# michaelbzms/DeepRecommendation

Measured on AMD Instinct MI355X. Metric: scored user-item pairs/sec, higher is better.
Workload: dtype f32; 1 GPU; cfg2: BasicNCF 1M users x 100k items, emb_dim=64, batch=65536/GPU, fp32, MLP 128-256-128-1; parallelism=replicas x1 (tables+MLP replicated, batch split, no collective), step_form=HIP-graph launches of 20 steps over the resident index batches, full=False

## Files before the change

deeprecommendation_amd/csrc/mlp_partial.hip:

```cpp
#include "mlp_fused.h"

#ifndef NCF_PART_WD
#define NCF_PART_WD 8
#endif
#ifndef NCF_PART_PF
#define NCF_PART_PF 2
#endif
#ifndef NCF_PART_HYBRID_MAX_PERMILLE
#define NCF_PART_HYBRID_MAX_PERMILLE 500
#endif

namespace ncf {

struct PartialBuildArgs {
    const float* tabA; int64_t rowsA; int64_t ldA; int QA;
    const float* Wp1; const float* b1;
    float* P; int64_t ldP;
};

template <int N1>
__global__ __launch_bounds__(256) void layer1_partial_kernel(PartialBuildArgs a) {
    constexpr int NT1 = N1 / 32;
    const int lane = threadIdx.x & 63;
    const int m = lane & 31, h = lane >> 5;
    const int64_t tile = (int64_t)blockIdx.x * 4 + (threadIdx.x >> 6);
    const int64_t rows = a.rowsA + 1;
    if (tile * 32 >= rows) return;
    const int64_t r = tile * 32 + m;
    const bool ok = r < a.rowsA;
    const float* rowA = a.tabA + (ok ? r : 0) * a.ldA + 4 * h;
    const float zA = ok ? 1.f : 0.f;

    f32x16 acc[NT1];
#pragma unroll
    for (int nt = 0; nt < NT1; ++nt)
#pragma unroll
        for (int g = 0; g < 4; ++g) {
            const f32x4 bb = fused_ldg4(a.b1 + 32 * nt + 8 * g + 4 * h);
            acc[nt][4 * g + 0] = bb[0]; acc[nt][4 * g + 1] = bb[1];
            acc[nt][4 * g + 2] = bb[2]; acc[nt][4 * g + 3] = bb[3];
        }
    const f32x4* wp = reinterpret_cast<const f32x4*>(a.Wp1) + lane;
    f32x4 w[NT1], x;
#pragma unroll
    for (int nt = 0; nt < NT1; ++nt) w[nt] = wp[nt * 64];
    x = fused_ldg4(rowA);
    for (int q = 0; q < a.QA; ++q) {
        f32x4 wn[NT1], xn;
        if (q + 1 < a.QA) {
#pragma unroll
            for (int nt = 0; nt < NT1; ++nt) wn[nt] = wp[((q + 1) * NT1 + nt) * 64];
            xn = fused_ldg4(rowA + 8 * (q + 1));
        }
        const f32x4 xb = x * zA;
#pragma unroll
        for (int nt = 0; nt < NT1; ++nt)
#pragma unroll
            for (int j = 0; j < 4; ++j)
                acc[nt] = __builtin_amdgcn_mfma_f32_32x32x2f32(w[nt][j], xb[j], acc[nt], 0, 0, 0);
#pragma unroll
        for (int nt = 0; nt < NT1; ++nt) w[nt] = wn[nt];
        x = xn;
    }
    if (r >= rows) return;
    float* dst = a.P + r * a.ldP + 4 * h;
#pragma unroll
    for (int nt = 0; nt < NT1; ++nt)
#pragma unroll
        for (int g = 0; g < 4; ++g) {
            f32x4 v;
            v[0] = acc[nt][4 * g + 0]; v[1] = acc[nt][4 * g + 1];
            v[2] = acc[nt][4 * g + 2]; v[3] = acc[nt][4 * g + 3];
            *reinterpret_cast<f32x4*>(dst + 32 * nt + 8 * g) = v;
        }
}

struct PartialArgs {
    const float* P; int64_t rowsA; int64_t ldP;
    const float* tabB; int64_t rowsB; int64_t ldB;
    const int64_t* idxA; const int64_t* idxB;
    int64_t B; int QA;
    const float* Wp1; const float* Wp2; const float* b2;
    const float* wl; const float* bl;
    float* out; int32_t* oob;
};

template <int QB, int N1, int N2>
__global__ __launch_bounds__(256, 2) void score_fused_partial_f32_kernel(PartialArgs a) {
    constexpr int NT1 = N1 / 32;
    constexpr int S = NT1 * QB;
    constexpr int WD0 = (QB >= 16 && N1 >= 256) ? 4 : NCF_PART_WD;
    constexpr int WD = WD0 < S ? WD0 : S;
    constexpr int PF = NCF_PART_PF < 1 ? 1 : (NCF_PART_PF < NT1 ? NCF_PART_PF : NT1);
    const int lane = threadIdx.x & 63;
    const int m = lane & 31, h = lane >> 5;
    const int64_t tile = (int64_t)blockIdx.x * 4 + (threadIdx.x >> 6);
    if (tile * 32 >= a.B) return;
    const int64_t p = tile * 32 + m;
    const int64_t pc = p < a.B ? p : a.B - 1;

    const int64_t ia = a.idxA ? a.idxA[pc] : pc;
    const int64_t ib = a.idxB ? a.idxB[pc] : pc;
    const bool okA = (ia >= 0) & (ia < a.rowsA), okB = (ib >= 0) & (ib < a.rowsB);
    if (!(okA & okB) && a.oob) *a.oob = 1;
    const float* prow = a.P + (okA ? ia : a.rowsA) * a.ldP + 4 * h;
    const float* rowB = a.tabB + (okB ? ib : 0) * a.ldB + 4 * h;
    const float zB = okB ? 1.f : 0.f;

    f32x16 acc1[NT1];
    auto load_p = [&](int nt) {
#pragma unroll
        for (int g = 0; g < 4; ++g) {
            const f32x4 v = fused_ldg4(prow + 32 * nt + 8 * g);
            acc1[nt][4 * g + 0] = v[0]; acc1[nt][4 * g + 1] = v[1];
            acc1[nt][4 * g + 2] = v[2]; acc1[nt][4 * g + 3] = v[3];
        }
    };
    const f32x4* wp = reinterpret_cast<const f32x4*>(a.Wp1) + (int64_t)a.QA * NT1 * 64 + lane;
    auto wfrag = [&](int s) { return wp[((s % QB) * NT1 + s / QB) * 64]; };
    f32x4 w[WD], x[QB];
    load_p(0);
#pragma unroll
    for (int s = 0; s < WD - 1; ++s) w[s] = wfrag(s);
#pragma unroll
    for (int t = 0; t < QB; ++t) x[t] = fused_ldg4(rowB + 8 * t);
#pragma unroll
    for (int nt = 1; nt < PF; ++nt) load_p(nt);
#pragma unroll
    for (int nt = 0; nt < NT1; ++nt) {
#pragma unroll
        for (int t = 0; t < QB; ++t) {
            const int s = nt * QB + t;
            const f32x4 xb = x[t] * zB;
#pragma unroll
            for (int j = 0; j < 4; ++j)
                acc1[nt] = __builtin_amdgcn_mfma_f32_32x32x2f32(w[s % WD][j], xb[j], acc1[nt], 0, 0, 0);
            if (s + WD - 1 < S) w[(s + WD - 1) % WD] = wfrag(s + WD - 1);
        }
        if (nt + PF < NT1) load_p(nt + PF);
#pragma unroll
        for (int t = 0; t < QB; ++t) {
            __builtin_amdgcn_sched_group_barrier(0x008, 4, 0);
            __builtin_amdgcn_sched_group_barrier(0x020, 1, 0);
        }
        __builtin_amdgcn_sched_group_barrier(0x020, 4, 0);
        __builtin_amdgcn_sched_barrier(0);
    }

    float score;
    if constexpr (N2 > 0) {
        f32x16 acc2[N2 / 32];
        fused_layer2<N1, N2>(acc1, acc2, a.b2, a.Wp2, lane);
        score = fused_last_layer(acc2, a.wl, a.bl, lane);
    } else {
        score = fused_last_layer(acc1, a.wl, a.bl, lane);
    }
    if (h == 0 && p < a.B) a.out[p] = score;
}

template <int QB, int N1, int N2>
static void launch_partial(const PartialArgs& a, hipStream_t s) {
    const int64_t tiles = (a.B + 31) / 32;
    hipLaunchKernelGGL((score_fused_partial_f32_kernel<QB, N1, N2>), dim3((unsigned)((tiles + 3) / 4)), dim3(256), 0, s, a);
}

#define NCF_PARTIAL_INSTANCES(X) \
    X(4, 256, 128) X(8, 256, 128) X(12, 256, 128) X(16, 256, 128) \
    X(4, 256, 0) X(8, 256, 0) X(12, 256, 0) X(16, 256, 0) \
    X(4, 128, 0) X(8, 128, 0) X(12, 128, 0) X(16, 128, 0) \
    X(4, 128, 64) X(8, 128, 64) X(12, 128, 64)

static bool partial_dispatch(int QB, int N1, int N2, const PartialArgs* a, hipStream_t s) {
#define X(qb, n1, n2) \
    if (QB == qb && N1 == n1 && N2 == n2) { if (a) launch_partial<qb, n1, n2>(*a, s); return true; }
    NCF_PARTIAL_INSTANCES(X)
#undef X
    return false;
}

static bool partial_shape_ok(int dtype, int EA, int EB, int n_layers, const int* dims) {
    if (dtype != NCF_F32 || !dims || EA <= 0 || EB <= 0 || EA % 8 || EB % 8) return false;
    if (!ncf_score_fused_supported(dtype, EA, EB, n_layers, dims)) return false;
    return partial_dispatch(EB / 8, dims[1], n_layers == 3 ? dims[2] : 0, nullptr, nullptr);
}

}

using namespace ncf;

extern "C" int ncf_score_fused_partial_supported(int dtype, int EA, int EB, int n_layers, const int* dims) {
    return partial_shape_ok(dtype, EA, EB, n_layers, dims) ? 1 : 0;
}

extern "C" int ncf_layer1_partial(int dtype, const void* tabA, int64_t rowsA, int64_t ldA, int EA, int EB, int n_layers,
                                  const int* dims, const void* packed, void* P, int64_t ldP, ncf_stream_t stream) {
    if (!partial_shape_ok(dtype, EA, EB, n_layers, dims))
        return fail(NCF_EUNSUPPORTED, "ncf_layer1_partial: no partial kernel for dtype=%d EA=%d EB=%d layers=%d", dtype, EA, EB, n_layers);
    const int N1 = dims[1];
    if (rowsA < 1 || !tabA || !packed || !P) return fail(NCF_EINVAL, "ncf_layer1_partial: bad argument");
    if (ldA < EA || ldA % 4 || ldP < N1 || ldP % 4 || !aligned16(tabA) || !aligned16(P) || !aligned16(packed))
        return fail(NCF_EINVAL, "ncf_layer1_partial: tables must be 16-byte aligned with ld %% 4 == 0");
    const BlobLayout L = blob_layout(dims, n_layers);
    PartialBuildArgs a;
    a.tabA = (const float*)tabA; a.rowsA = rowsA; a.ldA = ldA; a.QA = EA / 8;
    a.Wp1 = (const float*)packed + L.wp1; a.b1 = (const float*)packed + L.b1;
    a.P = (float*)P; a.ldP = ldP;
    const int64_t tiles = (rowsA + 1 + 31) / 32;
    const dim3 grid((unsigned)((tiles + 3) / 4)), block(256);
    if (N1 == 256) hipLaunchKernelGGL(layer1_partial_kernel<256>, grid, block, 0, (hipStream_t)stream, a);
    else hipLaunchKernelGGL(layer1_partial_kernel<128>, grid, block, 0, (hipStream_t)stream, a);
    return check_launch("ncf_layer1_partial");
}

extern "C" int ncf_score_fused_partial(int dtype, const void* P, int64_t ldP, const void* tabA, int64_t rowsA, int64_t ldA,
                                       const void* tabB, int64_t rowsB, int64_t ldB, const int64_t* idxA, const int64_t* idxB,
                                       int64_t B, int EA, int EB, int n_layers, const int* dims, const void* packed, float* out,
                                       int32_t* oob, ncf_stream_t stream) {
    if (!partial_shape_ok(dtype, EA, EB, n_layers, dims))
        return fail(NCF_EUNSUPPORTED, "ncf_score_fused_partial: no partial kernel for dtype=%d EA=%d EB=%d layers=%d", dtype, EA, EB, n_layers);
    if (B == 0) return NCF_OK;
    const int N1 = dims[1];
    if (B < 0 || rowsA < 1 || !P || !tabA || !tabB || !packed || !out) return fail(NCF_EINVAL, "ncf_score_fused_partial: bad argument");
    if (ldA < EA || ldB < EB || ldP < N1 || ldA % 4 || ldB % 4 || ldP % 4 || !aligned16(tabA) || !aligned16(tabB) || !aligned16(P) ||
        !aligned16(packed))
        return fail(NCF_EINVAL, "ncf_score_fused_partial: tables must be 16-byte aligned with ld %% 4 == 0");
    hipStream_t s = (hipStream_t)stream;
    auto plain = [&](int64_t off, int64_t n) {
        return ncf_score_fused(dtype, tabA, rowsA, ldA, tabB, rowsB, ldB, idxA ? idxA + off : nullptr, idxB ? idxB + off : nullptr,
                               n, EA, EB, n_layers, dims, packed, out + off, oob, stream);
    };
    const int64_t tiles = (B + 31) / 32;
    const int64_t round = 4 * (int64_t)num_cus();
    const int64_t full = tiles / round, rem = tiles % round;
    int64_t head = B;
    if (rem > 0 && rem * 1000 <= round * NCF_PART_HYBRID_MAX_PERMILLE && (full == 0 || (idxA && idxB))) head = full * round * 32;
    if (head == 0) return plain(0, B);
    const BlobLayout L = blob_layout(dims, n_layers);
    const float* pk = (const float*)packed;
    PartialArgs a;
    a.P = (const float*)P; a.rowsA = rowsA; a.ldP = ldP;
    a.tabB = (const float*)tabB; a.rowsB = rowsB; a.ldB = ldB;
    a.idxA = idxA; a.idxB = idxB; a.B = head; a.QA = EA / 8;
    a.Wp1 = pk + L.wp1;
    a.Wp2 = n_layers == 3 ? pk + L.wp2 : nullptr; a.b2 = n_layers == 3 ? pk + L.b2 : nullptr;
    a.wl = pk + L.wl; a.bl = pk + L.bl;
    a.out = out; a.oob = oob;
    partial_dispatch(EB / 8, N1, n_layers == 3 ? dims[2] : 0, &a, s);
    const int rc = check_launch("ncf_score_fused_partial");
    if (rc != NCF_OK || head == B) return rc;
    return plain(head, B - head);
}
```

deeprecommendation_amd/native.py:

```python
from __future__ import annotations

import ctypes
import os
from typing import Optional, Sequence

import torch

_HERE = os.path.dirname(os.path.abspath(__file__))
LIB_PATH = os.environ.get("NCF_HIP_LIBRARY") or os.path.join(_HERE, "libncf_hip.so")

NCF_F32, NCF_BF16 = 0, 1
NCF_OK, NCF_EINVAL, NCF_EUNSUPPORTED, NCF_ELAUNCH, NCF_EWORKSPACE = 0, -1, -2, -3, -4
ATT_MLP, ATT_LINEAR, ATT_COS, ATT_MLP_SCALED = 0, 1, 2, 3
ATT_SCALE_LOG2 = 64

_c_i64 = ctypes.c_int64
_c_p = ctypes.c_void_p
_c_int = ctypes.c_int
_c_size = ctypes.c_size_t

SIGNATURES = {
    "ncf_version": (_c_int, []),
    "ncf_last_error": (ctypes.c_char_p, []),
    "ncf_build_arch": (ctypes.c_char_p, []),
    "ncf_build_id": (ctypes.c_char_p, []),
    "ncf_probe_mfma_bf16": (_c_int, [_c_p, _c_int, _c_int, _c_int, _c_p, _c_p, _c_p]),
    "ncf_probe_copy": (_c_int, [_c_p, _c_p, _c_i64, _c_p]),
    "ncf_probe_gather_read": (_c_int, [_c_p, _c_i64, _c_i64, _c_int, _c_p, _c_i64, _c_int, _c_int, _c_p, _c_p]),
    "ncf_set_option": (_c_int, [ctypes.c_char_p, _c_int]),
    "ncf_get_option": (_c_int, [ctypes.c_char_p, _c_p]),
    "ncf_bucket_ids": (_c_int, [_c_p, _c_i64, _c_i64, _c_i64, _c_int, _c_i64, _c_p, _c_p, _c_p, _c_p, _c_p, _c_p]),
    "ncf_bucket_dedup_table_slots": (_c_size, [_c_i64]),
    "ncf_bucket_ids_dedup": (_c_int, [_c_p, _c_i64, _c_i64, _c_i64, _c_int, _c_i64, _c_p, _c_p, _c_i64, _c_p, _c_p, _c_p, _c_p, _c_p, _c_p]),
    "ncf_gather_buckets": (_c_int, [_c_int, _c_p, _c_i64, _c_i64, _c_p, _c_int, _c_i64, _c_int, _c_p, _c_i64, _c_p, _c_p]),
    "ncf_gather_concat": (_c_int, [_c_int, _c_p, _c_i64, _c_i64, _c_p, _c_i64, _c_i64, _c_p, _c_p, _c_i64, _c_int, _c_int,
                                   _c_p, _c_i64, _c_p, _c_p]),
    "ncf_gather_dot": (_c_int, [_c_int, _c_p, _c_i64, _c_i64, _c_p, _c_i64, _c_i64, _c_p, _c_p, _c_i64, _c_int, _c_p, _c_p, _c_p]),
    "ncf_mlp_workspace_bytes": (_c_size, [_c_int, _c_i64, _c_int, _c_p]),
    "ncf_mlp_forward": (_c_int, [_c_int, _c_p, _c_i64, _c_i64, _c_int, _c_p, _c_p, _c_p, _c_p, _c_size, _c_p, _c_i64, _c_p]),
    "ncf_score_fused_supported": (_c_int, [_c_int, _c_int, _c_int, _c_int, _c_p]),
    "ncf_mlp_packed_bytes": (_c_size, [_c_int, _c_int, _c_p]),
    "ncf_mlp_pack": (_c_int, [_c_int, _c_int, _c_p, _c_p, _c_p, _c_p, _c_size, _c_p]),
    "ncf_score_fused": (_c_int, [_c_int, _c_p, _c_i64, _c_i64, _c_p, _c_i64, _c_i64, _c_p, _c_p, _c_i64, _c_int, _c_int,
                                 _c_int, _c_p, _c_p, _c_p, _c_p, _c_p]),
    "ncf_spmm_csr": (_c_int, [_c_int, _c_p, _c_p, _c_i64, _c_p, _c_p, _c_p, _c_i64, _c_i64, _c_int, _c_p, _c_i64, _c_p,
                              _c_i64, _c_p, _c_int, _c_p]),
    "ncf_spmm_csr_dropout": (_c_int, [_c_int, _c_p, _c_p, _c_i64, _c_p, _c_p, _c_p, _c_i64, _c_i64, _c_int, _c_p, _c_i64, _c_p,
                                      _c_i64, _c_p, _c_int, _c_p, ctypes.c_uint32, ctypes.c_float, _c_p]),
    "ncf_degree_accumulate": (_c_int, [_c_p, _c_i64, _c_i64, _c_p, _c_p, _c_p]),
    "ncf_edge_coef": (_c_int, [_c_p, _c_p, _c_p, _c_p, _c_i64, _c_i64, _c_p, _c_p]),
    "ncf_scale_rows": (_c_int, [_c_p, _c_i64, _c_i64, _c_int, ctypes.c_float, _c_p, _c_i64, _c_p]),
    "ncf_attn_forward": (_c_int, [_c_int, _c_p, _c_i64, _c_p, _c_i64, _c_int, _c_p, ctypes.c_float, _c_p, _c_p, _c_p,
                                  _c_i64, _c_i64, _c_p, _c_i64, _c_int, _c_p, _c_p, _c_i64, _c_p, _c_p]),
    "ncf_attn_forward_dropout": (_c_int, [_c_int, _c_p, _c_i64, _c_p, _c_i64, _c_int, _c_p, ctypes.c_float, _c_p, _c_p, _c_p,
                                          _c_i64, _c_i64, _c_p, _c_i64, _c_int, _c_p, _c_p, _c_i64, _c_p, ctypes.c_uint32, ctypes.c_float, _c_p]),
    "ncf_attn_backward": (_c_int, [_c_int, _c_p, _c_i64, _c_p, _c_i64, _c_int, _c_p, _c_p, _c_p, _c_p, _c_i64, _c_i64, _c_p, _c_i64, _c_int,
                                   _c_p, _c_p, _c_i64, _c_p, _c_i64, _c_p, _c_i64, _c_p, _c_p, _c_i64, _c_p, ctypes.c_uint32, ctypes.c_float, _c_p]),
    "ncf_attn_forward_grouped": (_c_int, [_c_int, _c_p, _c_i64, _c_p, _c_i64, _c_int, _c_p, ctypes.c_float, _c_p, _c_p, _c_p,
                                          _c_i64, _c_i64, _c_p, _c_p, _c_p, _c_i64, _c_int, _c_p, _c_i64, _c_int, _c_p, _c_p,
                                          _c_i64, _c_p, _c_p, _c_p]),
    "ncf_group_pairs_workspace_bytes": (_c_size, [_c_i64]),
    "ncf_group_pairs": (_c_int, [_c_p, _c_i64, _c_i64, _c_int, _c_p, _c_p, _c_p, _c_p, _c_size, _c_p, _c_p]),
    "ncf_group_pairs_rows": (_c_int, [_c_p, _c_i64, _c_i64, _c_int, _c_p, _c_p, _c_p, _c_p, _c_p, _c_size, _c_p, _c_p]),
    "ncf_dense_csr_workspace_bytes": (_c_size, [_c_i64]),
    "ncf_dense_csr_rows": (_c_int, [_c_p, _c_i64, _c_i64, _c_i64, _c_int, _c_p, _c_p, _c_p, _c_size, _c_p]),
    "ncf_dense_csr_fill": (_c_int, [_c_p, _c_i64, _c_i64, _c_i64, _c_p, _c_p, _c_p, _c_p, _c_p]),
    "ncf_attn_candidates_supported": (_c_int, [_c_int, _c_int, _c_int]),
    "ncf_attn_candidates_workspace_bytes": (_c_size, [_c_i64]),
    "ncf_attn_candidates": (_c_int, [_c_p, _c_i64, _c_i64, _c_int, _c_p, _c_i64, _c_p, _c_int, _c_p, _c_p, _c_int, _c_p, _c_i64, _c_p, _c_i64,
                                     _c_p, _c_i64, _c_int, _c_p, _c_p, _c_p, _c_p, _c_p, _c_size, _c_p, _c_p]),
    "ncf_attn_candidates_pack_floats": (_c_size, [_c_int, _c_int]),
    "ncf_attn_candidates_packed_workspace_bytes": (_c_size, [_c_i64, _c_int, _c_i64]),
    "ncf_attn_candidates_pack": (_c_int, [_c_p, _c_i64, _c_int, _c_int, _c_p, _c_p]),
    "ncf_attn_candidates_packed": (_c_int, [_c_p, _c_i64, _c_i64, _c_int, _c_p, _c_p, _c_int, _c_p, _c_p, _c_int, _c_p, _c_i64, _c_p, _c_i64,
                                            _c_p, _c_i64, _c_int, _c_p, _c_p, _c_p, _c_p, _c_p, _c_size, _c_p, _c_p]),
    "ncf_attn_split_supported": (_c_int, [_c_int, _c_int, _c_int, _c_int]),
    "ncf_attn_split_workspace_bytes": (_c_size, [_c_i64, _c_int, _c_int]),
    "ncf_attn_forward_split": (_c_int, [_c_int, _c_p, _c_i64, _c_p, _c_i64, _c_int, _c_p, ctypes.c_float, _c_p, _c_p, _c_p,
                                        _c_i64, _c_i64, _c_p, _c_p, _c_p, _c_p, _c_i64, _c_int, _c_p, _c_i64, _c_int, _c_p, _c_p,
                                        _c_i64, _c_int, _c_int, _c_p, _c_size, _c_p]),
    "ncf_attn_tail_supported": (_c_int, [_c_int, _c_int, _c_int, _c_int]),
    "ncf_attn_tail_pack_weight": (_c_int, [_c_p, _c_int, _c_int, _c_p, _c_p]),
    "ncf_attn_tail": (_c_int, [_c_p, _c_i64, _c_int, _c_p, _c_int, _c_p, _c_i64, _c_int, _c_p, _c_p, _c_p, _c_int, _c_p, _c_p, _c_int,
                               _c_p, ctypes.c_float, _c_int, _c_p, _c_i64, _c_p]),
    "ncf_edge_softmax_csr": (_c_int, [_c_p, _c_p, _c_p, _c_p, _c_i64, _c_i64, _c_p, _c_p]),
    "ncf_edge_softmax_segmented_workspace_bytes": (_c_size, [_c_i64, _c_i64]),
    "ncf_edge_softmax_segmented": (_c_int, [_c_p, _c_p, _c_i64, _c_p, _c_i64, _c_p, _c_p, _c_p, _c_i64, _c_p, _c_p, _c_size, _c_p]),
    "ncf_score_fused_partial_supported": (_c_int, [_c_int, _c_int, _c_int, _c_int, _c_p]),
    "ncf_layer1_partial": (_c_int, [_c_int, _c_p, _c_i64, _c_i64, _c_int, _c_int, _c_int, _c_p, _c_p, _c_p, _c_i64, _c_p]),
    "ncf_score_fused_partial": (_c_int, [_c_int, _c_p, _c_i64, _c_p, _c_i64, _c_i64, _c_p, _c_i64, _c_i64, _c_p, _c_p, _c_i64,
                                         _c_int, _c_int, _c_int, _c_p, _c_p, _c_p, _c_p, _c_p]),
    "ncf_score_folded_supported": (_c_int, [_c_int, _c_int, _c_int]),
    "ncf_score_folded": (_c_int, [_c_int, _c_p, _c_i64, _c_i64, _c_p, _c_i64, _c_i64, _c_p, _c_p, _c_i64, _c_int, _c_int, _c_p,
                                  _c_p, _c_p, _c_p]),
    "ncf_linear_forward": (_c_int, [_c_int, _c_p, _c_i64, _c_i64, _c_p, _c_p, _c_int, _c_int, _c_int, _c_p, _c_i64, _c_p]),
    "ncf_gemm_tn_workspace_bytes": (_c_size, [_c_i64, _c_int, _c_int]),
    "ncf_gemm_tn": (_c_int, [_c_p, _c_i64, _c_p, _c_i64, _c_i64, _c_int, _c_int, _c_p, _c_i64, _c_p, _c_size, _c_p]),
    "ncf_colsum_workspace_bytes": (_c_size, [_c_i64, _c_int]),
    "ncf_colsum": (_c_int, [_c_p, _c_i64, _c_i64, _c_int, _c_p, _c_p, _c_size, _c_p]),
    "ncf_relu_backward": (_c_int, [_c_p, _c_i64, _c_p, _c_i64, _c_i64, _c_int, _c_p]),
    "ncf_relu_backward_out": (_c_int, [_c_p, _c_i64, _c_p, _c_i64, _c_p, _c_i64, _c_i64, _c_int, ctypes.c_float, _c_p]),
    "ncf_scatter_add_rows": (_c_int, [_c_p, _c_i64, _c_p, _c_i64, _c_int, _c_p, _c_i64, _c_i64, _c_p, _c_p]),
    "ncf_l2_normalize_rows": (_c_int, [_c_p, _c_i64, _c_i64, _c_int, _c_p, _c_i64, _c_p]),
    "ncf_gather_cols": (_c_int, [_c_p, _c_i64, _c_p, _c_p, _c_i64, _c_int, _c_i64, _c_p, _c_i64, _c_p, _c_p]),
    "ncf_scatter_add_cols": (_c_int, [_c_p, _c_i64, _c_p, _c_i64, _c_int, _c_p, _c_i64, _c_i64, _c_p, _c_p]),
    "ncf_topk_workspace_bytes": (_c_size, [_c_i64, _c_i64, _c_int]),
    "ncf_topk_rows": (_c_int, [_c_p, _c_i64, _c_i64, _c_i64, _c_p, _c_p, _c_int, _c_p, _c_p, _c_p, _c_p, _c_size, _c_p]),
    "ncf_dot_topk_workspace_bytes": (_c_size, [_c_i64, _c_i64, _c_int, _c_int]),
    "ncf_dot_topk": (_c_int, [_c_p, _c_i64, _c_i64, _c_p, _c_i64, _c_i64, _c_p, _c_p, _c_i64, _c_i64, _c_int, _c_p, _c_p, _c_int, _c_p,
                              _c_p, _c_p, _c_p, _c_size, _c_p, _c_p]),
    "ncf_mlp_topk_supported": (_c_int, [_c_int, _c_int, _c_int, _c_int, _c_p, _c_int]),
    "ncf_mlp_topk_workspace_bytes": (_c_size, [_c_i64, _c_i64, _c_int, _c_int, _c_p, _c_int]),
    "ncf_mlp_topk": (_c_int, [_c_int, _c_p, _c_i64, _c_i64, _c_p, _c_i64, _c_i64, _c_int, _c_int, _c_int, _c_p, _c_p, _c_i64, _c_i64,
                              _c_int, _c_p, _c_p, _c_p, _c_p, _c_int, _c_p, _c_p, _c_p, _c_p, _c_size, _c_p, _c_p]),
    "ncf_adam_step": (_c_int, [_c_p, _c_p, _c_p, _c_p, _c_i64, ctypes.c_float, ctypes.c_float, ctypes.c_float, ctypes.c_float,
                               ctypes.c_float, _c_i64, _c_p]),
    "ncf_negative_cdf": (_c_int, [_c_p, _c_i64, _c_p, ctypes.c_float, _c_p, _c_p, _c_p]),
    "ncf_sample_negatives": (_c_int, [_c_p, _c_p, _c_p, _c_i64, _c_p, _c_i64, ctypes.c_uint32, _c_i64, _c_p, _c_p, _c_p]),
}

_lib = None


class NativeError(RuntimeError):
    def __init__(self, code, msg):
        super().__init__(f"libncf_hip: {msg} (status {code})")
        self.code = code


def load_library(path: Optional[str] = None) -> ctypes.CDLL:
    global _lib
    if _lib is not None and path is None:
        return _lib
    p = path or LIB_PATH
    if not os.path.exists(p):
        raise RuntimeError(
            f"{p} not found: the HIP extension is not built. Run `python -c 'import __graft_entry__ as g; g.build()'` "
            "(needs hipcc). deeprecommendation_amd has no CPU fallback.")
    lib = ctypes.CDLL(p)
    for name, (res, args) in SIGNATURES.items():
        fn = getattr(lib, name)
        fn.restype = res
        fn.argtypes = args
    if path is None:
        if not os.environ.get("NCF_HIP_LIBRARY"):
            _check_build_id(lib, p)
        _lib = lib
        _options_from_environment(lib)
    return lib


def _check_build_id(lib, path):
    try:
        from .csrc import build as _build
        want = _build.source_id()
    except (ImportError, OSError):
        return
    have = lib.ncf_build_id().decode()
    if have != want:
        raise RuntimeError(f"{path} is stale: built from sources {have}, the sources here are {want}. "
                           "Rebuild: python -m deeprecommendation_amd.csrc.build")


OPTION_VALUES = {
    "bf16_kernel": {"auto": 0, "ws": 1, "stream": 2, "ws8": 3},
    "linear_kernel": {"auto": 0, "rs": 1, "rsp": 2},
    "linear_kslices": {"auto": 0, "4": 4, "8": 8},
    "attn_grouped_kernel": {"auto": 0, "lds": 1, "scalar": 2},
    "gather_kernel": {"auto": 0, "step": 1, "persistent": 2},
}
_ENV_OPTIONS = {"NCF_BF16_KERNEL": "bf16_kernel", "NCF_LINEAR_KERNEL": "linear_kernel", "NCF_LINEAR_KS": "linear_kslices",
# ... 186 lines not shown
def mlp_forward(x: torch.Tensor, weights: Sequence[torch.Tensor], biases: Sequence[Optional[torch.Tensor]],
                out: Optional[torch.Tensor] = None) -> torch.Tensor:
    lib = load_library()
    _dev(x, "x")
    if x.dtype != torch.float32:
        raise TypeError(f"mlp_forward computes in fp32; got activations of dtype {x.dtype}")
    B, K0, ldx = _rows2d(x, "x")
    dims = [K0] + [int(w.shape[0]) for w in weights]
    for i, w in enumerate(weights):
        _dev(w, "weight")
        if w.dtype != torch.float32 or not w.is_contiguous() or w.shape[1] != dims[i]:
            raise ValueError(f"weight {i} must be contiguous fp32 [{dims[i + 1]}, {dims[i]}]")
    biases = [None if b is None else b.contiguous() for b in biases]
    n = len(weights)
    d = _dims_array(dims)
    ws_bytes = lib.ncf_mlp_workspace_bytes(NCF_F32, B, n, d)
    ws = torch.empty(max(ws_bytes, 1), dtype=torch.uint8, device=x.device)
    if out is None:
        out = torch.empty((B, dims[-1]), dtype=torch.float32, device=x.device)
    _, _, ldo = _rows2d(out, "out")
    _check(lib.ncf_mlp_forward(NCF_F32, _ptr(x), B, ldx, n, d, _ptr_array(weights), _ptr_array(biases), _ptr(ws), ws_bytes,
                               _ptr(out), ldo, _stream(x)))
    return out


def linear(x: torch.Tensor, weight: torch.Tensor, bias: Optional[torch.Tensor] = None, out=None) -> torch.Tensor:
    return mlp_forward(x, [weight], [bias], out=out)


class PackedMLP:

    def __init__(self, weights: Sequence[torch.Tensor], biases: Sequence[Optional[torch.Tensor]], dtype=torch.float32):
        lib = load_library()
        self.dims = [int(weights[0].shape[1])] + [int(w.shape[0]) for w in weights]
        self.n_layers = len(weights)
        self.device = weights[0].device
        self.dtype = dtype
        self.dt = NCF_F32 if dtype == torch.float32 else NCF_BF16
        d = _dims_array(self.dims)
        nbytes = lib.ncf_mlp_packed_bytes(self.dt, self.n_layers, d)
        if nbytes == 0:
            raise NativeError(NCF_EUNSUPPORTED, "MLP shape cannot be packed for the fused kernel")
        ws = [w.detach().to(torch.float32).contiguous() for w in weights]
        bs = [None if b is None else b.detach().to(torch.float32).contiguous() for b in biases]
        for w in ws:
            _dev(w, "weight")
        self.blob = torch.empty(nbytes, dtype=torch.uint8, device=self.device)
        _check(lib.ncf_mlp_pack(self.dt, self.n_layers, d, _ptr_array(ws), _ptr_array(bs), _ptr(self.blob), nbytes,
                                _stream(ws[0])))

    def supports(self, EA: int, EB: int) -> bool:
        return bool(load_library().ncf_score_fused_supported(self.dt, EA, EB, self.n_layers, _dims_array(self.dims)))


def fused_supported(EA: int, EB: int, dims: Sequence[int], dtype=torch.float32) -> bool:
    dt = NCF_F32 if dtype == torch.float32 else NCF_BF16
    return bool(load_library().ncf_score_fused_supported(dt, EA, EB, len(dims) - 1, _dims_array(dims)))


def score_fused(tabA: torch.Tensor, idxA, tabB: Optional[torch.Tensor], idxB, packed: PackedMLP,
                out: Optional[torch.Tensor] = None, B: Optional[int] = None) -> torch.Tensor:
    lib = load_library()
    _dev(tabA, "tabA")
    rowsA, EA, ldA = _rows2d(tabA, "tabA")
    rowsB = EB = ldB = 0
    if tabB is not None:
        _dev(tabB, "tabB")
        rowsB, EB, ldB = _rows2d(tabB, "tabB")
    idxA, idxB = _idx(idxA), _idx(idxB)
    if B is None:
        B = idxA.numel() if idxA is not None else (idxB.numel() if idxB is not None else rowsA)
    if out is None:
        out = torch.empty((B, 1), dtype=torch.float32, device=tabA.device)
    if tabA.dtype != packed.dtype:
        raise TypeError(f"tables are {tabA.dtype} but the MLP was packed for {packed.dtype}")
    _check(lib.ncf_score_fused(_dt(tabA), _ptr(tabA), rowsA, ldA, _ptr(tabB), rowsB, ldB, _ptr(idxA), _ptr(idxB), B, EA, EB,
                               packed.n_layers, _dims_array(packed.dims), _ptr(packed.blob), _ptr(out),
                               _ptr(_oob_flag(tabA.device)), _stream(tabA)))
    return out


def partial_supported(EA: int, EB: int, packed: PackedMLP) -> bool:
    return packed.dt == NCF_F32 and bool(load_library().ncf_score_fused_partial_supported(
        NCF_F32, int(EA), int(EB), packed.n_layers, _dims_array(packed.dims)))


def layer1_partial(tabA: torch.Tensor, packed: PackedMLP, out: Optional[torch.Tensor] = None) -> torch.Tensor:
    lib = load_library()
    _dev(tabA, "tabA")
    rowsA, EA, ldA = _rows2d(tabA, "tabA")
    EB, N1 = packed.dims[0] - EA, packed.dims[1]
    if out is None:
        out = torch.empty((rowsA + 1, N1), dtype=torch.float32, device=tabA.device)
    if out.shape[0] < rowsA + 1 or out.shape[1] < N1:
        raise ValueError(f"layer1_partial: out must hold ({rowsA + 1}, {N1}) floats")
    _, _, ldP = _rows2d(out, "out")
    _check(lib.ncf_layer1_partial(_dt(tabA), _ptr(tabA), rowsA, ldA, EA, EB, packed.n_layers, _dims_array(packed.dims),
                                  _ptr(packed.blob), _ptr(out), ldP, _stream(tabA)))
    return out


def score_fused_partial(P: torch.Tensor, tabA: torch.Tensor, idxA, tabB: torch.Tensor, idxB, packed: PackedMLP,
                        out: Optional[torch.Tensor] = None, B: Optional[int] = None) -> torch.Tensor:
    lib = load_library()
    _dev(tabA, "tabA"), _dev(tabB, "tabB"), _dev(P, "P")
    rowsA, EA, ldA = _rows2d(tabA, "tabA")
    rowsB, EB, ldB = _rows2d(tabB, "tabB")
    _, _, ldP = _rows2d(P, "P")
    if P.dtype != torch.float32 or P.shape[0] != rowsA + 1 or P.shape[1] != packed.dims[1]:
        raise ValueError(f"P must be fp32 ({rowsA + 1}, {packed.dims[1]}), built by layer1_partial from this tabA")
    idxA, idxB = _idx(idxA), _idx(idxB)
    if B is None:
        B = idxA.numel() if idxA is not None else (idxB.numel() if idxB is not None else rowsA)
    if out is None:
        out = torch.empty((B, 1), dtype=torch.float32, device=tabA.device)
    if tabA.dtype != packed.dtype:
        raise TypeError(f"tables are {tabA.dtype} but the MLP was packed for {packed.dtype}")
    _check(lib.ncf_score_fused_partial(_dt(tabA), _ptr(P), ldP, _ptr(tabA), rowsA, ldA, _ptr(tabB), rowsB, ldB, _ptr(idxA),
                                       _ptr(idxB), B, EA, EB, packed.n_layers, _dims_array(packed.dims), _ptr(packed.blob),
                                       _ptr(out), _ptr(_oob_flag(tabA.device)), _stream(tabA)))
    return out


def spmm_csr(segptr: torch.Tensor, row_of: Optional[torch.Tensor], col: torch.Tensor, coef: Optional[torch.Tensor],
             z: torch.Tensor, N: int, y: Optional[torch.Tensor] = None, acc_sum: Optional[torch.Tensor] = None,
             partial: Optional[torch.Tensor] = None, fixup: bool = True, dropout: Optional[tuple] = None) -> torch.Tensor:
    lib = load_library()
    _dev(z, "z")
    Nz, D, ldz = _rows2d(z, "z")
    n_seg = segptr.numel() - 1
    if segptr.dtype != torch.int64 or col.dtype != torch.int32:
        raise TypeError("segptr must be int64 and col int32")
    if row_of is not None and row_of.dtype != torch.int32:
        raise TypeError("row_of must be int32")
    if y is None:
        y = torch.empty((N, D), dtype=torch.float32, device=z.device)
    if row_of is not None and partial is None:
        partial = torch.empty((n_seg, D), dtype=torch.float32, device=z.device)
    if dropout is not None and dropout[0] > 0:
        p, seed, eid = dropout
        if eid is not None and (eid.dtype != torch.int32 or eid.numel() != col.numel()):
            raise TypeError("edge ids must be int32, one per CSR entry")
        _check(lib.ncf_spmm_csr_dropout(NCF_F32, _ptr(segptr), _ptr(row_of), n_seg, _ptr(col), _ptr(coef), _ptr(z), Nz, ldz, D, _ptr(y),
                                        y.stride(0), _ptr(acc_sum), 0 if acc_sum is None else acc_sum.stride(0), _ptr(partial),
                                        1 if fixup else 0, _ptr(eid), int(seed) & 0xFFFFFFFF, float(p), _stream(z)))
        return y
    _check(lib.ncf_spmm_csr(NCF_F32, _ptr(segptr), _ptr(row_of), n_seg, _ptr(col), _ptr(coef), _ptr(z), Nz, ldz, D, _ptr(y),
                            y.stride(0), _ptr(acc_sum), 0 if acc_sum is None else acc_sum.stride(0), _ptr(partial),
                            1 if fixup else 0, _stream(z)))
    return y


class SegmentedCSR:

    def __init__(self, rowptr: torch.Tensor, col: torch.Tensor, coef: Optional[torch.Tensor], seg_len: int = 512, fan: int = 64):
        self.n_rows = rowptr.numel() - 1
        self.col, self.coef = col, coef
        counts = rowptr[1:] - rowptr[:-1]
        self._build_tree(rowptr, counts, seg_len, fan)

    @staticmethod
    def _split(rowptr, row_ids, counts, seg_len):
        dev = rowptr.device
        nseg = torch.clamp((counts + seg_len - 1) // seg_len, min=1)
        n = counts.numel()
        if n == 0 or int(nseg.max()) == 1:
# ... 730 lines not shown
```

include/ncf_abi.h:

```cpp
#ifndef NCF_ABI_H
#define NCF_ABI_H

#include <stddef.h>
#include <stdint.h>

#ifdef __cplusplus
extern "C" {
#endif

#define NCF_ABI_VERSION 1

typedef void* ncf_stream_t;

enum ncf_dtype { NCF_F32 = 0, NCF_BF16 = 1 };

enum ncf_status {
    NCF_OK = 0,
    NCF_EINVAL = -1,
    NCF_EUNSUPPORTED = -2,
    NCF_ELAUNCH = -3,
    NCF_EWORKSPACE = -4
};

int ncf_version(void);
const char* ncf_last_error(void);
const char* ncf_build_arch(void);
const char* ncf_build_id(void);

int ncf_set_option(const char* name, int value);
int ncf_get_option(const char* name, int* value);

int ncf_gather_concat(int dtype,
                      const void* dev_tabA, int64_t rowsA, int64_t ldA,
                      const void* dev_tabB, int64_t rowsB, int64_t ldB,
                      const int64_t* dev_idxA, const int64_t* dev_idxB,
                      int64_t B, int EA, int EB,
                      void* dev_out, int64_t ldOut,
                      int32_t* dev_oob_flag, ncf_stream_t stream);

int ncf_gather_dot(int dtype,
                   const void* dev_tabA, int64_t rowsA, int64_t ldA,
                   const void* dev_tabB, int64_t rowsB, int64_t ldB,
                   const int64_t* dev_idxA, const int64_t* dev_idxB,
                   int64_t B, int E, float* dev_out,
                   int32_t* dev_oob_flag, ncf_stream_t stream);

int ncf_bucket_ids(const int64_t* dev_idx, int64_t B, int64_t rows_per_rank, int64_t total_rows, int world, int64_t cap,
                   int64_t* dev_send, int64_t* dev_slot, int32_t* dev_counts,
                   int32_t* dev_oob_flag, int32_t* dev_overflow_flag, ncf_stream_t stream);

size_t ncf_bucket_dedup_table_slots(int64_t B);
int ncf_bucket_ids_dedup(const int64_t* dev_idx, int64_t B, int64_t rows_per_rank, int64_t total_rows, int world, int64_t cap,
                         int64_t* dev_hkeys, int64_t* dev_hvals, int64_t table_slots,
                         int64_t* dev_send, int64_t* dev_slot, int32_t* dev_counts,
                         int32_t* dev_oob_flag, int32_t* dev_overflow_flag, ncf_stream_t stream);

int ncf_gather_buckets(int dtype, const void* dev_table, int64_t rows, int64_t ld, const int64_t* dev_recv, int world, int64_t cap, int E,
                       void* dev_out, int64_t ldout, int32_t* dev_oob_flag, ncf_stream_t stream);

size_t ncf_mlp_workspace_bytes(int dtype, int64_t B, int n_layers, const int* dims);
int ncf_mlp_forward(int dtype, const void* dev_x, int64_t B, int64_t ldx,
                    int n_layers, const int* dims,
                    const void* const* host_W, const void* const* host_b,
                    void* dev_workspace, size_t workspace_bytes,
                    void* dev_out, int64_t ldOut, ncf_stream_t stream);

int ncf_score_fused_supported(int dtype, int EA, int EB, int n_layers, const int* dims);
size_t ncf_mlp_packed_bytes(int dtype, int n_layers, const int* dims);
int ncf_mlp_pack(int dtype, int n_layers, const int* dims,
                 const void* const* host_W, const void* const* host_b,
                 void* dev_packed, size_t packed_bytes, ncf_stream_t stream);
int ncf_score_fused(int dtype,
                    const void* dev_tabA, int64_t rowsA, int64_t ldA,
                    const void* dev_tabB, int64_t rowsB, int64_t ldB,
                    const int64_t* dev_idxA, const int64_t* dev_idxB,
                    int64_t B, int EA, int EB,
                    int n_layers, const int* dims, const void* dev_packed,
                    float* dev_out, int32_t* dev_oob_flag, ncf_stream_t stream);

int ncf_score_fused_partial_supported(int dtype, int EA, int EB, int n_layers, const int* dims);
int ncf_layer1_partial(int dtype, const void* dev_tabA, int64_t rowsA, int64_t ldA, int EA, int EB,
                       int n_layers, const int* dims, const void* dev_packed,
                       void* dev_P, int64_t ldP, ncf_stream_t stream);
int ncf_score_fused_partial(int dtype, const void* dev_P, int64_t ldP,
                            const void* dev_tabA, int64_t rowsA, int64_t ldA,
                            const void* dev_tabB, int64_t rowsB, int64_t ldB,
                            const int64_t* dev_idxA, const int64_t* dev_idxB,
                            int64_t B, int EA, int EB,
                            int n_layers, const int* dims, const void* dev_packed,
                            float* dev_out, int32_t* dev_oob_flag, ncf_stream_t stream);

int ncf_score_folded_supported(int dtype, int N1, int N2);
int ncf_score_folded(int dtype,
                     const void* dev_PA, int64_t rowsA, int64_t ldPA,
                     const void* dev_PB, int64_t rowsB, int64_t ldPB,
                     const int64_t* dev_idxA, const int64_t* dev_idxB,
                     int64_t B, int N1, int N2, const void* dev_packed_tail,
                     float* dev_out, int32_t* dev_oob_flag, ncf_stream_t stream);

int ncf_spmm_csr(int dtype, const int64_t* dev_segptr, const int32_t* dev_row_of, int64_t n_seg,
                 const int32_t* dev_col, const float* dev_coef,
                 const void* dev_z, int64_t Nz, int64_t ldz, int D,
                 void* dev_y, int64_t ldy, float* dev_sum, int64_t ldsum,
                 float* dev_partial, int fixup, ncf_stream_t stream);

int ncf_spmm_csr_dropout(int dtype, const int64_t* dev_segptr, const int32_t* dev_row_of, int64_t n_seg,
                         const int32_t* dev_col, const float* dev_coef,
                         const void* dev_z, int64_t Nz, int64_t ldz, int D,
                         void* dev_y, int64_t ldy, float* dev_sum, int64_t ldsum,
                         float* dev_partial, int fixup, const int32_t* dev_edge_id, uint32_t seed, float p, ncf_stream_t stream);

int ncf_degree_accumulate(const int64_t* dev_dst, int64_t E, int64_t N, float* dev_deg,
                          int32_t* dev_oob_flag, ncf_stream_t stream);
int ncf_edge_coef(const int64_t* dev_src, const int64_t* dev_dst, const float* dev_attr,
                  const float* dev_deg, int64_t E, int64_t N, float* dev_coef, ncf_stream_t stream);
int ncf_edge_softmax_csr(const int64_t* dev_rowptr, const int32_t* dev_col, const float* dev_attr, const float* dev_s,
                         int64_t n_rows, int64_t Ns, float* dev_out, ncf_stream_t stream);
size_t ncf_edge_softmax_segmented_workspace_bytes(int64_t n_seg, int64_t n_rows);
int ncf_edge_softmax_segmented(const int64_t* dev_segptr, const int32_t* dev_row_of, int64_t n_seg, const int64_t* dev_seg_first,
                               int64_t n_rows, const int32_t* dev_col, const float* dev_attr, const float* dev_s, int64_t n_src,
                               float* dev_out, void* dev_workspace, size_t workspace_bytes, ncf_stream_t stream);

int ncf_scale_rows(const float* dev_in, int64_t ldin, int64_t N, int D, float divisor,
                   float* dev_out, int64_t ldout, ncf_stream_t stream);

enum ncf_att_mode { NCF_ATT_MLP = 0, NCF_ATT_LINEAR = 1, NCF_ATT_COS = 2, NCF_ATT_MLP_SCALED = 3 };
#define NCF_ATT_SCALE_LOG2 64
int ncf_attn_forward(int mode,
                     const float* dev_pc, int64_t ldpc, const float* dev_pr, int64_t ldpr, int A,
                     const float* dev_w1, float b1,
                     const int64_t* dev_rowptr, const int32_t* dev_col, const float* dev_val,
                     int64_t B, int64_t I,
                     const float* dev_feat, int64_t ldfeat, int Fdim,
                     const float* dev_out_bias,
                     float* dev_out_feat, int64_t ldout,
                     float* dev_weights,
                     ncf_stream_t stream);

int ncf_attn_forward_dropout(int mode,
                             const float* dev_pc, int64_t ldpc, const float* dev_pr, int64_t ldpr, int A,
                             const float* dev_w1, float b1,
                             const int64_t* dev_rowptr, const int32_t* dev_col, const float* dev_val,
                             int64_t B, int64_t I,
                             const float* dev_feat, int64_t ldfeat, int Fdim, const float* dev_out_bias,
                             float* dev_out_feat, int64_t ldout, float* dev_weights,
                             uint32_t seed, float p, ncf_stream_t stream);
int ncf_attn_backward(int mode,
                      const float* dev_pc, int64_t ldpc, const float* dev_pr, int64_t ldpr, int A, const float* dev_w1,
                      const int64_t* dev_rowptr, const int32_t* dev_col, const float* dev_val, int64_t B, int64_t I,
                      const float* dev_feat, int64_t ldfeat, int Fdim,
                      const float* dev_weights, const float* dev_dout, int64_t lddout,
                      float* dev_d_pc, int64_t ldd_pc, float* dev_d_pr, int64_t ldd_pr, float* dev_d_w1_part,
                      float* dev_d_feat, int64_t ldd_feat, float* dev_scratch,
                      uint32_t seed, float p, ncf_stream_t stream);

int ncf_attn_forward_grouped(int mode,
                             const float* dev_pc, int64_t ldpc, const float* dev_pr, int64_t ldpr, int A,
                             const float* dev_w1, float b1,
                             const int64_t* dev_rowptr, const int32_t* dev_col, const float* dev_val,
                             int64_t n_rows, int64_t n_rated,
                             const int64_t* dev_grp_ptr, const int64_t* dev_pair_ids, const int64_t* dev_wg_ptr,
                             int64_t B, int pairs_per_wg,
                             const float* dev_feat, int64_t ldfeat, int Fdim, const float* dev_out_bias,
// ... 119 lines not shown
```

Baseline: 1.061 billion pairs/s.

## Stage layer-1 B-side weight fragments in LDS for partial fused scoring kernel

For shapes where QB*N1/32 <= 80, each block cooperatively loads the B-half of the packed layer-1 weights into shared memory once, then each wave streams fragments from LDS with a 2-deep register ring instead of re-reading them from global/L2 per wave. This is meant to cut the repeated global weight-fragment traffic and free registers held by the deeper global prefetch window. In exchange it adds an LDS allocation (up to 80 KB per block), a block barrier, and early-exit waves must stay alive until the barrier, which may reduce occupancy. An ablation macro and a query entry point are also added.

New measurement: 1.146 billion pairs/s (median of 6 runs). +8.0%, better.

```diff
diff --git a/deeprecommendation_amd/csrc/mlp_partial.hip b/deeprecommendation_amd/csrc/mlp_partial.hip
--- a/deeprecommendation_amd/csrc/mlp_partial.hip
+++ b/deeprecommendation_amd/csrc/mlp_partial.hip
@@ -5,6 +5,15 @@
 #endif
 #ifndef NCF_PART_PF
 #define NCF_PART_PF 2
+#endif
+#ifndef NCF_PART_LDS
+#define NCF_PART_LDS 1
+#endif
+#ifndef NCF_PART_LDS_PF
+#define NCF_PART_LDS_PF 2
+#endif
+#ifndef NCF_PART_ABLATE
+#define NCF_PART_ABLATE 0
 #endif
 #ifndef NCF_PART_HYBRID_MAX_PERMILLE
 #define NCF_PART_HYBRID_MAX_PERMILLE 500
@@ -85,25 +94,39 @@
     float* out; int32_t* oob;
 };
 
-template <int QB, int N1, int N2>
+constexpr bool partial_in_lds(int QB, int N1) { return NCF_PART_LDS && QB * (N1 / 32) <= 80; }
+
+template <int QB, int N1, int N2, bool LDS>
 __global__ __launch_bounds__(256, 2) void score_fused_partial_f32_kernel(PartialArgs a) {
     constexpr int NT1 = N1 / 32;
     constexpr int S = NT1 * QB;
     constexpr int WD0 = (QB >= 16 && N1 >= 256) ? 4 : NCF_PART_WD;
-    constexpr int WD = WD0 < S ? WD0 : S;
-    constexpr int PF = NCF_PART_PF < 1 ? 1 : (NCF_PART_PF < NT1 ? NCF_PART_PF : NT1);
-    const int lane = threadIdx.x & 63;
+    constexpr int WD = LDS ? 2 : (WD0 < S ? WD0 : S);
+    constexpr int PF0 = LDS ? NCF_PART_LDS_PF : NCF_PART_PF;
+    constexpr int PF = PF0 < 1 ? 1 : (PF0 < NT1 ? PF0 : NT1);
+    constexpr int FILL = LDS ? S / 4 : 1;
+    constexpr bool ABL_P = (NCF_PART_ABLATE & 1) != 0, ABL_W = (NCF_PART_ABLATE & 2) != 0;
+    __shared__ __attribute__((aligned(16))) f32x4 wlds[LDS ? S * 64 : 1];
+    const int lane = threadIdx.x & 63, wave = threadIdx.x >> 6;
     const int m = lane & 31, h = lane >> 5;
-    const int64_t tile = (int64_t)blockIdx.x * 4 + (threadIdx.x >> 6);
-    if (tile * 32 >= a.B) return;
+    const int64_t tile = (int64_t)blockIdx.x * 4 + wave;
+    const bool live = tile * 32 < a.B;
+    if (!LDS && !live) return;
     const int64_t p = tile * 32 + m;
     const int64_t pc = p < a.B ? p : a.B - 1;
 
     const int64_t ia = a.idxA ? a.idxA[pc] : pc;
     const int64_t ib = a.idxB ? a.idxB[pc] : pc;
+    const f32x4* wp = reinterpret_cast<const f32x4*>(a.Wp1) + (int64_t)a.QA * NT1 * 64 + lane;
+    auto wfrag = [&](int s) { return wp[((s % QB) * NT1 + s / QB) * 64]; };
+    f32x4 fill[FILL];
+    if constexpr (LDS) {
+#pragma unroll
+        for (int i = 0; i < FILL; ++i) fill[i] = wp[(((4 * i) % QB + wave) * NT1 + (4 * i) / QB) * 64];
+    }
     const bool okA = (ia >= 0) & (ia < a.rowsA), okB = (ib >= 0) & (ib < a.rowsB);
-    if (!(okA & okB) && a.oob) *a.oob = 1;
-    const float* prow = a.P + (okA ? ia : a.rowsA) * a.ldP + 4 * h;
+    if (!(okA & okB) && a.oob && live) *a.oob = 1;
+    const float* prow = a.P + ((okA && !ABL_P) ? ia : a.rowsA) * a.ldP + 4 * h;
     const float* rowB = a.tabB + (okB ? ib : 0) * a.ldB + 4 * h;
     const float zB = okB ? 1.f : 0.f;
 
@@ -116,16 +139,26 @@
             acc1[nt][4 * g + 2] = v[2]; acc1[nt][4 * g + 3] = v[3];
         }
     };
-    const f32x4* wp = reinterpret_cast<const f32x4*>(a.Wp1) + (int64_t)a.QA * NT1 * 64 + lane;
-    auto wfrag = [&](int s) { return wp[((s % QB) * NT1 + s / QB) * 64]; };
     f32x4 w[WD], x[QB];
     load_p(0);
-#pragma unroll
-    for (int s = 0; s < WD - 1; ++s) w[s] = wfrag(s);
+    if constexpr (!LDS) {
+#pragma unroll
+        for (int s = 0; s < WD - 1; ++s) w[s] = wfrag(s);
+    }
 #pragma unroll
     for (int t = 0; t < QB; ++t) x[t] = fused_ldg4(rowB + 8 * t);
 #pragma unroll
     for (int nt = 1; nt < PF; ++nt) load_p(nt);
+    const f32x4* wq = wlds + lane;
+    if constexpr (LDS) {
+#pragma unroll
+        for (int i = 0; i < FILL; ++i) wlds[(4 * i + wave) * 64 + lane] = fill[i];
+        __syncthreads();
+        if (!live) return;
+        w[0] = wq[0];
+        w[1] = wq[64];
+        __builtin_amdgcn_sched_barrier(0);
+    }
 #pragma unroll
     for (int nt = 0; nt < NT1; ++nt) {
 #pragma unroll
@@ -135,13 +168,19 @@
 #pragma unroll
             for (int j = 0; j < 4; ++j)
                 acc1[nt] = __builtin_amdgcn_mfma_f32_32x32x2f32(w[s % WD][j], xb[j], acc1[nt], 0, 0, 0);
-            if (s + WD - 1 < S) w[(s + WD - 1) % WD] = wfrag(s + WD - 1);
+            if constexpr (LDS) {
+                if (s + 2 < S && !ABL_W) w[s % 2] = wq[(s + 2) * 64];
+            } else {
+                if (s + WD - 1 < S) w[(s + WD - 1) % WD] = ABL_W ? w[s % WD] : wfrag(s + WD - 1);
+            }
         }
         if (nt + PF < NT1) load_p(nt + PF);
-#pragma unroll
-        for (int t = 0; t < QB; ++t) {
-            __builtin_amdgcn_sched_group_barrier(0x008, 4, 0);
-            __builtin_amdgcn_sched_group_barrier(0x020, 1, 0);
+        if (!ABL_W) {
+#pragma unroll
+            for (int t = 0; t < QB; ++t) {
+                __builtin_amdgcn_sched_group_barrier(0x008, 4, 0);
+                __builtin_amdgcn_sched_group_barrier(LDS ? 0x100 : 0x020, 1, 0);
+            }
         }
         __builtin_amdgcn_sched_group_barrier(0x020, 4, 0);
         __builtin_amdgcn_sched_barrier(0);
@@ -161,7 +200,7 @@
 template <int QB, int N1, int N2>
 static void launch_partial(const PartialArgs& a, hipStream_t s) {
     const int64_t tiles = (a.B + 31) / 32;
-    hipLaunchKernelGGL((score_fused_partial_f32_kernel<QB, N1, N2>), dim3((unsigned)((tiles + 3) / 4)), dim3(256), 0, s, a);
+    hipLaunchKernelGGL((score_fused_partial_f32_kernel<QB, N1, N2, partial_in_lds(QB, N1)>), dim3((unsigned)((tiles + 3) / 4)), dim3(256), 0, s, a);
 }
 
 #define NCF_PARTIAL_INSTANCES(X) \
@@ -190,6 +229,10 @@
 
 extern "C" int ncf_score_fused_partial_supported(int dtype, int EA, int EB, int n_layers, const int* dims) {
     return partial_shape_ok(dtype, EA, EB, n_layers, dims) ? 1 : 0;
+}
+
+extern "C" int ncf_score_fused_partial_in_lds(int dtype, int EA, int EB, int n_layers, const int* dims) {
+    return partial_shape_ok(dtype, EA, EB, n_layers, dims) && partial_in_lds(EB / 8, dims[1]) ? 1 : 0;
 }
 
 extern "C" int ncf_layer1_partial(int dtype, const void* tabA, int64_t rowsA, int64_t ldA, int EA, int EB, int n_layers,
diff --git a/deeprecommendation_amd/native.py b/deeprecommendation_amd/native.py
--- a/deeprecommendation_amd/native.py
+++ b/deeprecommendation_amd/native.py
@@ -87,6 +87,7 @@
     "ncf_edge_softmax_segmented_workspace_bytes": (_c_size, [_c_i64, _c_i64]),
     "ncf_edge_softmax_segmented": (_c_int, [_c_p, _c_p, _c_i64, _c_p, _c_i64, _c_p, _c_p, _c_p, _c_i64, _c_p, _c_p, _c_size, _c_p]),
     "ncf_score_fused_partial_supported": (_c_int, [_c_int, _c_int, _c_int, _c_int, _c_p]),
+    "ncf_score_fused_partial_in_lds": (_c_int, [_c_int, _c_int, _c_int, _c_int, _c_p]),
     "ncf_layer1_partial": (_c_int, [_c_int, _c_p, _c_i64, _c_i64, _c_int, _c_int, _c_int, _c_p, _c_p, _c_p, _c_i64, _c_p]),
     "ncf_score_fused_partial": (_c_int, [_c_int, _c_p, _c_i64, _c_p, _c_i64, _c_i64, _c_p, _c_i64, _c_i64, _c_p, _c_p, _c_i64,
                                          _c_int, _c_int, _c_int, _c_p, _c_p, _c_p, _c_p, _c_p]),
@@ -439,6 +440,11 @@
 
 def partial_supported(EA: int, EB: int, packed: PackedMLP) -> bool:
     return packed.dt == NCF_F32 and bool(load_library().ncf_score_fused_partial_supported(
+        NCF_F32, int(EA), int(EB), packed.n_layers, _dims_array(packed.dims)))
+
+
+def partial_in_lds(EA: int, EB: int, packed: PackedMLP) -> bool:
+    return packed.dt == NCF_F32 and bool(load_library().ncf_score_fused_partial_in_lds(
         NCF_F32, int(EA), int(EB), packed.n_layers, _dims_array(packed.dims)))
 
 
diff --git a/include/ncf_abi.h b/include/ncf_abi.h
--- a/include/ncf_abi.h
+++ b/include/ncf_abi.h
@@ -79,6 +79,7 @@
                     float* dev_out, int32_t* dev_oob_flag, ncf_stream_t stream);
 
 int ncf_score_fused_partial_supported(int dtype, int EA, int EB, int n_layers, const int* dims);
+int ncf_score_fused_partial_in_lds(int dtype, int EA, int EB, int n_layers, const int* dims);
 int ncf_layer1_partial(int dtype, const void* dev_tabA, int64_t rowsA, int64_t ldA, int EA, int EB,
                        int n_layers, const int* dims, const void* dev_packed,
                        void* dev_P, int64_t ldP, ncf_stream_t stream);
```
